# FluxML/Flux3D.jl

Hardware: AMD Instinct MI355X
Metric: chamfer_point_pairs_per_sec (higher is better)
Workload: dtype f32

## Files before the change

flux3d.jl_amd/csrc/chamfer.hip:

```cpp
#include <cmath>
#include <type_traits>

#include "nn1_common.h"

using namespace fx3d;

#ifdef FX3D_PROBE
__device__ unsigned long long g_probe[4096 * 16];
#define FX3D_PROBE_MARK(k)                                                                   \
    do {                                                                                     \
        if (threadIdx.x == 0 && blockIdx.x < 4096) {                                         \
            g_probe[blockIdx.x * 16 + (k)] = __builtin_readcyclecounter();                   \
            if ((k) == 0) g_probe[blockIdx.x * 16 + 13] = wall_clock64();                    \
            if ((k) == 12) g_probe[blockIdx.x * 16 + 14] = wall_clock64();                   \
        }                                                                                    \
    } while (0)
__device__ unsigned long long g_probe2[256 * 16];
#define FX3D_PROBE_MARK2(k) do { if (threadIdx.x == 0 && blockIdx.x < 256) g_probe2[blockIdx.x * 16 + (k)] = __builtin_readcyclecounter(); } while (0)
__device__ unsigned long long g_probe3[16 * 16 * 8];
#define FX3D_PROBE_MARKW(k) do { if ((threadIdx.x & 63) == 0 && blockIdx.x < 16) g_probe3[(blockIdx.x * 16 + (threadIdx.x >> 6)) * 8 + (k)] = __builtin_readcyclecounter(); } while (0)
#else
#define FX3D_PROBE_MARK(k) do { } while (0)
#define FX3D_PROBE_MARK2(k) do { } while (0)
#define FX3D_PROBE_MARKW(k) do { } while (0)
#endif

namespace {

__device__ __forceinline__ void load4pts(const float *__restrict__ base, int p0, float (&px)[4],
                                         float (&py)[4], float (&pz)[4]) {
    const float4 *s4 = reinterpret_cast<const float4 *>(base + (size_t)p0 * 3);
    const float4 f0 = s4[0], f1 = s4[1], f2 = s4[2];
    px[0] = f0.x; py[0] = f0.y; pz[0] = f0.z;
    px[1] = f0.w; py[1] = f1.x; pz[1] = f1.y;
    px[2] = f1.z; py[2] = f1.w; pz[2] = f2.x;
    px[3] = f2.y; py[3] = f2.z; pz[3] = f2.w;
}

typedef _Float16 h8 __attribute__((ext_vector_type(8)));
typedef float f32x16 __attribute__((ext_vector_type(16)));
#ifndef FX3D_HFIFO
#define FX3D_HFIFO 5
#endif
constexpr int kHFifo = FX3D_HFIFO;
#ifndef FX3D_HRUNS_FROM
#define FX3D_HRUNS_FROM 16
#endif
constexpr int kHRunsFrom = FX3D_HRUNS_FROM;
constexpr int kScanU = 2;
#ifndef FX3D_HRUNCAP
#define FX3D_HRUNCAP 384
#endif
constexpr int kHRunCap = FX3D_HRUNCAP;
constexpr int kHItemCap = 64 * kHFifo > kHRunCap ? 64 * kHFifo : kHRunCap;
constexpr int kHFarCap = 64;
#ifndef FX3D_HBLKTRACK
#define FX3D_HBLKTRACK 1
#endif
constexpr bool kHBlkTrack = FX3D_HBLKTRACK != 0;
constexpr int kHIdBits = kHBlkTrack ? 7 : 6;
static_assert(kHChunkMax / (32 * kHLT) <= 64, "lane-tile ids live in the six (block ids: seven) low mantissa bits of the tracked keys");
constexpr float kKeyUp = kHBlkTrack ? 0x1.2p-16f : 0x1.2p-17f;
constexpr float kPadF16 = 65504.0f;
__device__ const unsigned short kHilbertCell[512] = {
    0, 1, 65, 64, 72, 73, 9, 8, 16, 24, 88, 80, 81, 89, 25, 17, 18, 26, 27, 19, 83, 91, 90, 82, 74, 10, 11, 75, 67, 3, 2, 66,
    130, 194, 195, 131, 139, 203, 202, 138, 146, 154, 155, 147, 211, 219, 218, 210, 209, 217, 153, 145, 144, 152, 216, 208, 200, 201, 137, 136, 128, 129, 193, 192,
    256, 257, 265, 264, 328, 329, 321, 320, 384, 448, 456, 392, 393, 457, 449, 385, 386, 450, 451, 387, 395, 459, 458, 394, 330, 322, 323, 331, 267, 259, 258, 266,
    274, 282, 283, 275, 339, 347, 346, 338, 402, 466, 467, 403, 411, 475, 474, 410, 409, 473, 465, 401, 400, 464, 472, 408, 344, 345, 337, 336, 272, 273, 281, 280,
    288, 296, 297, 289, 353, 361, 360, 352, 416, 480, 481, 417, 425, 489, 488, 424, 432, 496, 504, 440, 441, 505, 497, 433, 369, 368, 376, 377, 313, 312, 304, 305,
    306, 307, 315, 314, 378, 379, 371, 370, 434, 498, 506, 442, 443, 507, 499, 435, 427, 491, 490, 426, 418, 482, 483, 419, 355, 363, 362, 354, 290, 298, 299, 291,
    227, 235, 171, 163, 162, 170, 234, 226, 225, 224, 160, 161, 169, 168, 232, 233, 241, 240, 248, 249, 185, 184, 176, 177, 178, 242, 250, 186, 187, 251, 243, 179,
    115, 51, 59, 123, 122, 58, 50, 114, 113, 112, 120, 121, 57, 56, 48, 49, 41, 40, 104, 105, 97, 96, 32, 33, 34, 42, 106, 98, 99, 107, 43, 35,
    36, 44, 108, 100, 101, 109, 45, 37, 38, 39, 103, 102, 110, 111, 47, 46, 54, 55, 63, 62, 126, 127, 119, 118, 117, 53, 61, 125, 124, 60, 52, 116,
    180, 244, 252, 188, 189, 253, 245, 181, 182, 183, 191, 190, 254, 255, 247, 246, 238, 239, 175, 174, 166, 167, 231, 230, 229, 237, 173, 165, 164, 172, 236, 228,
    292, 300, 301, 293, 357, 365, 364, 356, 420, 484, 485, 421, 429, 493, 492, 428, 436, 500, 508, 444, 445, 509, 501, 437, 373, 372, 380, 381, 317, 316, 308, 309,
    310, 311, 319, 318, 382, 383, 375, 374, 438, 502, 510, 446, 447, 511, 503, 439, 431, 495, 494, 430, 422, 486, 487, 423, 359, 367, 366, 358, 294, 302, 303, 295,
    287, 286, 278, 279, 343, 342, 350, 351, 415, 479, 471, 407, 406, 470, 478, 414, 413, 477, 476, 412, 404, 468, 469, 405, 341, 349, 348, 340, 276, 284, 285, 277,
    269, 261, 260, 268, 332, 324, 325, 333, 397, 461, 460, 396, 388, 452, 453, 389, 390, 454, 462, 398, 399, 463, 455, 391, 327, 326, 334, 335, 271, 270, 262, 263,
    199, 198, 134, 135, 143, 142, 206, 207, 215, 223, 159, 151, 150, 158, 222, 214, 213, 221, 220, 212, 148, 156, 157, 149, 141, 205, 204, 140, 132, 196, 197, 133,
    69, 5, 4, 68, 76, 12, 13, 77, 85, 93, 92, 84, 20, 28, 29, 21, 22, 30, 94, 86, 87, 95, 31, 23, 15, 14, 78, 79, 71, 70, 6, 7,
};
constexpr size_t kHScratchBytes = (kHThreads / 64) * (32 * 8 + kHItemCap * 2 + 32 * 3 * 4) + 64 * 32;

__device__ __forceinline__ float vmin(float a, float b) {
    float r;
    asm("v_min_f32 %0, %1, %2" : "=v"(r) : "v"(a), "v"(b));
    return r;
}

__device__ __forceinline__ float vmax(float a, float b) {
    float r;
    asm("v_max_f32 %0, %1, %2" : "=v"(r) : "v"(a), "v"(b));
    return r;
}

__device__ __forceinline__ void split2h(float v, _Float16 &h, _Float16 &l) {
    h = (_Float16)v;
    l = (_Float16)(v - (float)h);
}

constexpr float kBetaC = 0x1.1p-18f;
constexpr float kBandB1 = 1.0f + 18.0f * kBetaC + 0x1p-20f;
constexpr float kBandA = 22.3f * kBetaC + 0x1p-19f;
__device__ __forceinline__ void make_pieces(float cx, float cy, float cz, h8 &p0, h8 &p1) {
    _Float16 hx, lx, hy, ly, hz, lz, n1, n2, n3;
    split2h(cx, hx, lx); split2h(cy, hy, ly); split2h(cz, hz, lz);
    const float n0 = ((cx * cx) + (cy * cy)) + (cz * cz);
    const float n = n0 + kBetaC * n0;
    n1 = (_Float16)n;
    const float r1 = n - (float)n1;
    n2 = (_Float16)r1;
    n3 = (_Float16)(r1 - (float)n2);
    const _Float16 z = (_Float16)0.0f;
    p0 = h8{hx, hx, lx, hy, hy, ly, hz, hz};
    p1 = h8{lz, n1, n2, n3, lx, ly, lz, z};
}

template <bool WANT_IDX, bool SPLITFUSE = false, bool PRUNE = false>
__global__ __launch_bounds__(kHThreads, 4) void nn1_f16_kernel(Nn1Params p) {
    extern __shared__ __attribute__((aligned(16))) float lds[];
    __shared__ __attribute__((aligned(16))) float red[4 * 4 * (kHThreads / 64) + 16];
    __shared__ int nfar[2];
    __shared__ unsigned short farlist[kHFarCap];
    constexpr int QB = (kHThreads / 64) * 32;

    const int L = blockIdx.x;
    const int nsplit = PRUNE ? 1 : p.nsplit;
    const int per_cloud = p.tiles * nsplit;
    const bool by_xcd = 2 * p.B >= 8;
    const int slot = by_xcd ? L >> 3 : L;
    const int c = by_xcd ? (slot / per_cloud) * 8 + (L & 7) : slot / per_cloud;
    const int tile = (slot % per_cloud) / nsplit;
    const int split = (slot % per_cloud) % nsplit;
    if (c >= 2 * p.B) return;
    const int dir = c >= p.B ? 1 : 0;
    const int b = dir ? c - p.B : c;
    const int NQ = dir ? p.M : p.N;
    const int NC = dir ? p.N : p.M;
    if (tile >= (dir ? p.tiles_y : p.tiles_x)) return;
    if ((long long)split * p.chunk >= NC) return;
    const int ctail = (!PRUNE && p.tail > 0 && nsplit == 1 && NC > p.chunk && NC - p.chunk <= p.tail) ? NC - p.chunk : 0;
    const int NCm = NC - ctail;
    const float *__restrict__ qb = (dir ? p.y : p.x) + (size_t)b * NQ * 3;
    const float *__restrict__ cb = (dir ? p.x : p.y) + (size_t)b * NC * 3;
    int32_t *idx_out = dir ? p.idx_y : p.idx_x;
    float *dmin_out = dir ? p.dmin_y : p.dmin_x;

    const int tid = threadIdx.x, lane = tid & 63;
    const int wv = __builtin_amdgcn_readfirstlane(tid >> 6);
    const int jq = lane & 31, hh = lane >> 5;
    const int CH = p.chunk;
    const int tpb = dir ? p.tpb_y : p.tpb;
    h8 *imgp = reinterpret_cast<h8 *>(lds);
    float4 *imgf = reinterpret_cast<float4 *>(lds);
    unsigned long long *wres = reinterpret_cast<unsigned long long *>(lds + 8 * (CH + 64));
    unsigned short *witems = reinterpret_cast<unsigned short *>(wres + (kHThreads / 64) * 32);
    float *wq = reinterpret_cast<float *>(witems + (kHThreads / 64) * kHItemCap);
    unsigned long long *qres = wres + wv * 32;
    unsigned short *items = witems + wv * kHItemCap;
    float *qtab = wq + wv * 96;
    const bool vec = (reinterpret_cast<uintptr_t>(cb) & 15) == 0;
    const bool one_shot = PRUNE || NCm <= CH;
    if (tid == 0) { nfar[0] = 0; nfar[1] = 0; }
    float qpre[3];
    {
        const int q0i = (tile * tpb) * QB + wv * 32 + jq;
        const int qc0 = q0i < NQ ? q0i : NQ - 1;
#pragma unroll
        for (int d = 0; d < 3; ++d) qpre[d] = qb[(size_t)qc0 * 3 + d];
    }
    if constexpr (PRUNE) {
        unsigned int *zc = reinterpret_cast<unsigned int *>(wres);
        for (int i = tid; i < 1040 + 16 * 256; i += kHThreads) zc[i] = 0u;
        int *gb = reinterpret_cast<int *>(wq + (kHThreads / 64) * 96) + 64 * 8;
        for (int i = tid; i < kHGroupsMax * 8; i += kHThreads) gb[i] = (i & 4) ? (int)0x80000000 : 0x7fffffff;
    }
    FX3D_PROBE_MARK(0);

    const bool own_chunk_only = nsplit > 1 && (long long)split * CH + (long long)nsplit * CH >= NCm;
    const int s_lo = own_chunk_only ? split * CH : 0;
    const int SN = own_chunk_only ? (NCm - s_lo < CH ? NCm - s_lo : CH) : NC;
    const float *__restrict__ sb = cb + (size_t)s_lo * 3;
    const bool parked = one_shot || own_chunk_only;
    float mu[3], cinf = 0.0f, varmax = 0.0f;
    float bxlo[3] = {0.f, 0.f, 0.f}, bxhi[3] = {0.f, 0.f, 0.f};
    bool allfin = true;
    {
        float mn[3] = {INFINITY, INFINITY, INFINITY}, mx[3] = {-INFINITY, -INFINITY, -INFINITY}, sm3[3] = {0.f, 0.f, 0.f};
        float sqt = 0.0f;
        const float pil[3] = {sb[0], sb[1], sb[2]};
        const int nsweep = (SN + kHThreads - 1) / kHThreads;
        for (int i0 = 0; i0 < nsweep; i0 += 4) {
            P3 v[4];
#pragma unroll
            for (int e = 0; e < 4; ++e) {
                const int pt = (i0 + e) * kHThreads + tid;
                v[e] = *reinterpret_cast<const P3 *>(sb + (size_t)(pt < SN ? pt : SN - 1) * 3);
            }
#pragma unroll
            for (int e = 0; e < 4; ++e) {
                const int pt = (i0 + e) * kHThreads + tid;
                mn[0] = fminf(mn[0], v[e].x); mx[0] = fmaxf(mx[0], v[e].x);
                mn[1] = fminf(mn[1], v[e].y); mx[1] = fmaxf(mx[1], v[e].y);
                mn[2] = fminf(mn[2], v[e].z); mx[2] = fmaxf(mx[2], v[e].z);
                if (pt < SN) {
                    sm3[0] = sm3[0] + v[e].x; sm3[1] = sm3[1] + v[e].y; sm3[2] = sm3[2] + v[e].z;
                    if (parked) imgf[((pt >> 5) * 2) * 32 + (pt & 31)] = float4{v[e].x, v[e].y, v[e].z, 0.0f};
                }
                if (((i0 + e) & 3) == (wv & 3) && pt < SN) {
                    sqt = __builtin_fmaf(v[e].x - pil[0], v[e].x - pil[0], sqt); sqt = __builtin_fmaf(v[e].y - pil[1], v[e].y - pil[1], sqt);
                    sqt = __builtin_fmaf(v[e].z - pil[2], v[e].z - pil[2], sqt);
                }
            }
        }
        FX3D_PROBE_MARK(5);
        {
            float4 lo4, hi4, st4;
            lo4.x = wave_min_l63(mn[0]); lo4.y = wave_min_l63(mn[1]); lo4.z = wave_min_l63(mn[2]); lo4.w = 0.0f;
            hi4.x = wave_max_l63(mx[0]); hi4.y = wave_max_l63(mx[1]); hi4.z = wave_max_l63(mx[2]); hi4.w = 0.0f;
            st4.x = wave_sum_l63(sm3[0]); st4.y = wave_sum_l63(sm3[1]); st4.z = wave_sum_l63(sm3[2]); st4.w = wave_sum_l63(sqt);
            if (lane == 63) {
                float4 *r4 = reinterpret_cast<float4 *>(red);
                r4[wv * 4] = lo4; r4[wv * 4 + 1] = hi4; r4[wv * 4 + 2] = st4;
            }
        }
        FX3D_PROBE_MARK(9);
        __syncthreads();
        FX3D_PROBE_MARK(10);
        static_assert(kHThreads / 64 == 16, "the cross-wave reduction below: one wave's row of 16 lanes, one lane per wave");
        if (wv == 0) {
            const float4 *r4 = reinterpret_cast<const float4 *>(red);
            const int w = lane & 15;
            float4 lo4 = r4[w * 4], hi4 = r4[w * 4 + 1], st4 = r4[w * 4 + 2];
#define NN1_ROW_MIN(v) v = fkey_inv(row_mm_key<false>(fkey(v)));
#define NN1_ROW_MAX(v) v = fkey_inv(row_mm_key<true>(fkey(v)));
#define NN1_ROW_SUM(v) v = v + dpp_mov<0xB1>(v); v = v + dpp_mov<0x4E>(v); v = v + dpp_mov<0x141>(v); v = v + dpp_mov<0x140>(v);
            NN1_ROW_MIN(lo4.x) NN1_ROW_MIN(lo4.y) NN1_ROW_MIN(lo4.z)
            NN1_ROW_MAX(hi4.x) NN1_ROW_MAX(hi4.y) NN1_ROW_MAX(hi4.z)
            NN1_ROW_SUM(st4.x) NN1_ROW_SUM(st4.y) NN1_ROW_SUM(st4.z) NN1_ROW_SUM(st4.w)
#undef NN1_ROW_MIN
#undef NN1_ROW_MAX
#undef NN1_ROW_SUM
            const float lo3[3] = {lo4.x, lo4.y, lo4.z}, hi3[3] = {hi4.x, hi4.y, hi4.z}, st3[3] = {st4.x, st4.y, st4.z};
            float m3[3], ci = 0.0f, vm = st4.w / fmaxf(0.25f * (float)SN, 1.0f);
            bool fin = true;
#pragma unroll
            for (int d = 0; d < 3; ++d) {
                const float lo = lo3[d], hi = hi3[d], st = st3[d];
                m3[d] = fminf(fmaxf(st / (float)SN, lo), hi);
                const float off = st / (float)SN - pil[d];
                vm = vm - off * off;
                ci = fmaxf(ci, fmaxf(hi - m3[d], m3[d] - lo));
                fin = fin && fabsf(st) < INFINITY;
            }
            if (lane == 0) {
                float4 *o4 = reinterpret_cast<float4 *>(red) + 4 * (kHThreads / 64);
                o4[0] = float4{m3[0], m3[1], m3[2], ci * 1.000001f};
                o4[1] = float4{vm, fin ? 1.0f : 0.0f, 0.0f, 0.0f};
                if (PRUNE) { o4[2] = float4{lo3[0], lo3[1], lo3[2], 0.0f}; o4[3] = float4{hi3[0], hi3[1], hi3[2], 0.0f}; }
            }
        }
        __syncthreads();
        {
            const float4 *o4 = reinterpret_cast<const float4 *>(red) + 4 * (kHThreads / 64);
            const float4 a = o4[0], b2 = o4[1];
            mu[0] = a.x; mu[1] = a.y; mu[2] = a.z; cinf = a.w;
            varmax = b2.x; allfin = b2.y != 0.0f;
            if (PRUNE) {
                const float4 l4 = o4[2], h4 = o4[3];
                bxlo[0] = l4.x; bxlo[1] = l4.y; bxlo[2] = l4.z; bxhi[0] = h4.x; bxhi[1] = h4.y; bxhi[2] = h4.z;
            }
        }
    }
    float rng = cinf;
    if (allfin && cinf < 1.0e16f && 3.0f * cinf * cinf > kRobustGate * varmax) {
        const float4 r = robust_range3<kHThreads, false>(sb, SN, parked, imgf, red, mu[0], mu[1], mu[2], cinf);
        mu[0] = r.x; mu[1] = r.y; mu[2] = r.z; rng = r.w;
    }
    const bool sane = allfin && cinf < 1.0e16f;
    float sc = 1.0f;
    if (sane && rng > 1.0e-30f) {
        int e;
        (void)frexpf(rng, &e);
        sc = ldexpf(1.0f, 7 - e);
    }
    auto uni = [](float v) { return __builtin_bit_cast(float, __builtin_amdgcn_readfirstlane(__builtin_bit_cast(int, v))); };
    mu[0] = uni(mu[0]); mu[1] = uni(mu[1]); mu[2] = uni(mu[2]); sc = uni(sc); rng = uni(rng); cinf = uni(cinf);
    const bool has_far = sane && rng < cinf;
    int fslot = 0;
    auto pieces = [&](float x, float y, float z, int pt, h8 &p0, h8 &p1) {
        const float sx = (x - mu[0]) * sc, sy = (y - mu[1]) * sc, sz = (z - mu[2]) * sc;
        if (!has_far) { make_pieces(sx, sy, sz, p0, p1); return; }
        const bool far = !(fmaxf(fmaxf(fabsf(sx), fabsf(sy)), fabsf(sz)) < 128.0f);
        make_pieces(far ? 0.f : sx, far ? 0.f : sy, far ? 0.f : sz, p0, p1);
        if (far) {
            p1[7] = (_Float16)kPadF16;
            const int f = atomicAdd(&nfar[fslot], 1);
            if (f < kHFarCap) farlist[f] = (unsigned short)pt;
        }
    };

    [[maybe_unused]] float4 *cs = nullptr, *qsw = nullptr;
    [[maybe_unused]] bool sorted_c = false;
    [[maybe_unused]] int qwlen = 0;
    [[maybe_unused]] float4 *boxes = nullptr;
    if constexpr (PRUNE) {
        cs = p.pscr + (size_t)blockIdx.x * p.pscr_stride;
        qsw = cs + kHChunkMax;
        boxes = reinterpret_cast<float4 *>(wq + (kHThreads / 64) * 96);
        unsigned int *ccnt = reinterpret_cast<unsigned int *>(wres);
        unsigned int *qtot = ccnt + 520;
        unsigned int *qwh = qtot + 520;
        const bool last_t = tile == (dir ? p.tiles_y : p.tiles_x) - 1;
        const int qw0 = tile * tpb * QB;
        const int qw1 = last_t || qw0 + tpb * QB > NQ ? NQ : qw0 + tpb * QB;
        qwlen = qw1 - qw0;
        const int cnt = NCm;
        const bool do_sort = sane && cnt >= 512;
        const bool sorted_q = do_sort && NQ <= 4 * kHThreads;
        P3 qv[4];
        if (sorted_q) {
#pragma unroll
            for (int e = 0; e < 4; ++e) {
                const int qp = 256 * wv + 64 * e + lane;
                qv[e] = *reinterpret_cast<const P3 *>(qb + (size_t)(qp < NQ ? qp : NQ - 1) * 3);
            }
        }
        FX3D_PROBE_MARK2(0);
        int *gbox = reinterpret_cast<int *>(boxes + 64 * 2);
        auto group_box = [&](int wrow, float x, float y, float z) {
            int *g = gbox + (wrow >> 5) * 8;
            atomicMin(g + 0, fkey((x - mu[0]) * sc)); atomicMin(g + 1, fkey((y - mu[1]) * sc)); atomicMin(g + 2, fkey((z - mu[2]) * sc));
            atomicMax(g + 4, fkey((x - mu[0]) * sc)); atomicMax(g + 5, fkey((y - mu[1]) * sc)); atomicMax(g + 6, fkey((z - mu[2]) * sc));
        };
        if (do_sort) {
            float4 cv[4];
#pragma unroll
            for (int e = 0; e < 4; ++e) {
                const int pt = e * kHThreads + tid;
                cv[e] = float4{0.f, 0.f, 0.f, 0.f};
                if (pt < cnt) cv[e] = imgf[((pt >> 5) * 2) * 32 + (pt & 31)];
            }
            FX3D_PROBE_MARK2(1);
            float inv[3], off[3], cfl[3], cfh[3];
#pragma unroll
            for (int d = 0; d < 3; ++d) {
                const float fr = has_far ? 0.125f * rng : 128.0f / sc;
                const float flo = fmaxf(bxlo[d], mu[d] - fr), fhi = fminf(bxhi[d], mu[d] + fr);
                inv[d] = fhi > flo ? 8.0f / (fhi - flo) : 0.0f;
                off[d] = -flo * inv[d];
                cfl[d] = flo; cfh[d] = fhi;
            }
            auto cell = [&](float x, float y, float z) -> unsigned int {
                const unsigned int ux = (unsigned int)(int)fminf(fmaxf(__builtin_fmaf(x, inv[0], off[0]), 0.0f), 7.0f);
                const unsigned int uy = (unsigned int)(int)fminf(fmaxf(__builtin_fmaf(y, inv[1], off[1]), 0.0f), 7.0f);
                const unsigned int uz = (unsigned int)(int)fminf(fmaxf(__builtin_fmaf(z, inv[2], off[2]), 0.0f), 7.0f);
                return ux | (uy << 3) | (uz << 6);
            };

            unsigned int ccr[4], qcr[4];
            auto count_cells = [&](bool valid, unsigned int t, auto &&add) -> unsigned int {
                unsigned int rank = 0u;
                bool mine = valid;
                const unsigned int tn = (unsigned int)__builtin_amdgcn_update_dpp((int)~t, (int)t, 0x111, 0xF, 0xF, false);
                if (__builtin_popcountll(__ballot(valid && t == tn)) >= 8) {
                    unsigned long long rem = __ballot(valid);
                    for (int it = 0; it < 12 && rem; ++it) {
                        const unsigned int t0 = (unsigned int)__builtin_amdgcn_readlane((int)t, __builtin_ctzll(rem));
                        const unsigned long long grp = __ballot(mine && t == t0);
                        rem &= ~grp;
                        if (__builtin_popcountll(grp) < 4) continue;
                        unsigned int base = 0u;
                        if ((int)lane == __builtin_ctzll(grp)) base = add(t0, (unsigned int)__builtin_popcountll(grp));
                        base = (unsigned int)__builtin_amdgcn_readlane((int)base, __builtin_ctzll(grp));
                        if (mine && t == t0) {
                            rank = base + __builtin_amdgcn_mbcnt_hi((unsigned int)(grp >> 32), __builtin_amdgcn_mbcnt_lo((unsigned int)grp, 0u));
                            mine = false;
                        }
                    }
                }
                if (mine) rank = add(t, 1u);
                return rank;
            };
#pragma unroll
            for (int e = 0; e < 4; ++e) {
                const int pt = e * kHThreads + tid;
                const unsigned int t = pt < cnt ? cell(cv[e].x, cv[e].y, cv[e].z) : 0u;
                ccr[e] = (t << 16) | count_cells(pt < cnt, t, [&](unsigned int c, unsigned int n) { return atomicAdd(&ccnt[c], n); });
            }
            int *qbb = reinterpret_cast<int *>(boxes + 64 * 2 + kHGroupsMax * 2 - 2);
            if (sorted_q) {
                int kl[3] = {0x7fffffff, 0x7fffffff, 0x7fffffff}, kh[3] = {(int)0x80000000, (int)0x80000000, (int)0x80000000};
#pragma unroll
                for (int e = 0; e < 4; ++e) {
                    const int qp = 256 * wv + 64 * e + lane;
                    if (qp < NQ) {
                        const int k3[3] = {fkey(qv[e].x), fkey(qv[e].y), fkey(qv[e].z)};
#pragma unroll
                        for (int d = 0; d < 3; ++d) { kl[d] = kl[d] < k3[d] ? kl[d] : k3[d]; kh[d] = kh[d] > k3[d] ? kh[d] : k3[d]; }
                    }
                }
#pragma unroll
                for (int d = 0; d < 3; ++d) {
                    int a = row_mm_key<false>(kl[d]), b2 = row_mm_key<true>(kh[d]);
                    a = imm<false>(a, dpp_keepi<0x142, 0xA>(a)); a = imm<false>(a, dpp_keepi<0x143, 0xC>(a));
                    b2 = imm<true>(b2, dpp_keepi<0x142, 0xA>(b2)); b2 = imm<true>(b2, dpp_keepi<0x143, 0xC>(b2));
                    if (lane == 63) { atomicMin(qbb + d, a); atomicMax(qbb + 4 + d, b2); }
                }
            }
            FX3D_PROBE_MARK2(2);
            __syncthreads();
            FX3D_PROBE_MARK2(3);
            float qinv[3] = {0.f, 0.f, 0.f}, qoff[3] = {0.f, 0.f, 0.f};
            if (sorted_q) {
                const float ext = fmaxf(fmaxf(cfh[0] - cfl[0], cfh[1] - cfl[1]), cfh[2] - cfl[2]);
#pragma unroll
                for (int d = 0; d < 3; ++d) {
                    const float ql = fkey_inv(qbb[d]), qh = fkey_inv(qbb[4 + d]);
                    const float grow = qh - ql > 4.0f * ext ? 0.25f * ext : ext;
                    const float lo = fmaxf(ql, cfl[d] - grow), hi = fminf(qh, cfh[d] + grow);
                    qinv[d] = hi > lo && hi - lo < INFINITY ? 8.0f / (hi - lo) : 0.0f;
                    qoff[d] = qinv[d] != 0.0f ? -lo * qinv[d] : 0.0f;
                }
            }
            auto qcell = [&](float x, float y, float z) -> unsigned int {
                const unsigned int ux = (unsigned int)(int)fminf(fmaxf(__builtin_fmaf(x, qinv[0], qoff[0]), 0.0f), 7.0f);
                const unsigned int uy = (unsigned int)(int)fminf(fmaxf(__builtin_fmaf(y, qinv[1], qoff[1]), 0.0f), 7.0f);
                const unsigned int uz = (unsigned int)(int)fminf(fmaxf(__builtin_fmaf(z, qinv[2], qoff[2]), 0.0f), 7.0f);
                return ux | (uy << 3) | (uz << 6);
            };
            auto curve_scan = [&](unsigned int *a) {
                unsigned int tc[8];
                {
                    const uint4 h = *reinterpret_cast<const uint4 *>(kHilbertCell + 8 * lane);
                    tc[0] = h.x & 0xffffu; tc[1] = h.x >> 16; tc[2] = h.y & 0xffffu; tc[3] = h.y >> 16;
                    tc[4] = h.z & 0xffffu; tc[5] = h.z >> 16; tc[6] = h.w & 0xffffu; tc[7] = h.w >> 16;
                }
                unsigned int c8[8], tot = 0u;
#pragma unroll
                for (int k = 0; k < 8; ++k) { c8[k] = a[tc[k]]; tot += c8[k]; }
                unsigned int inc = tot;
#pragma unroll
                for (int o = 1; o < 64; o <<= 1) {
                    const unsigned int v = __shfl_up(inc, o, 64);
                    if (lane >= o) inc += v;
                }
                unsigned int run = inc - tot;
#pragma unroll
                for (int k = 0; k < 8; ++k) { a[tc[k]] = run; run += c8[k]; }
            };
            if (wv == 0) curve_scan(ccnt);
            if (sorted_q) {
#pragma unroll
                for (int e = 0; e < 4; ++e) {
                    const int qp = 256 * wv + 64 * e + lane;
                    const unsigned int t = qp < NQ ? qcell(qv[e].x, qv[e].y, qv[e].z) : 0u;
                    qcr[e] = (t << 16) | count_cells(qp < NQ, t, [&](unsigned int c, unsigned int n) {
                                 const unsigned int sh = 16u * (c & 1u);
                                 const unsigned int old = atomicAdd(&qwh[wv * 256 + (c >> 1)], n << sh);
                                 atomicAdd(&qtot[c], n);
                                 return (old >> sh) & 0xffffu;
                             });
                }
            }
            FX3D_PROBE_MARK2(4);
            __syncthreads();
            FX3D_PROBE_MARK2(5);
#pragma unroll
            for (int e = 0; e < 4; ++e) {
                const int pt = e * kHThreads + tid;
                if (pt < cnt) {
                    const int pos = (int)(ccnt[ccr[e] >> 16] + (ccr[e] & 0xffffu));
                    imgf[((pos >> 5) * 2) * 32 + (pos & 31)] = float4{cv[e].x, cv[e].y, cv[e].z, __builtin_bit_cast(float, pt)};
                }
            }
            sorted_c = true;
            if (sorted_q) {
                if (wv == 1) {
                    curve_scan(qtot);
                } else if (wv >= 2 && wv < 6) {
// ... 22 lines not shown
                            group_box(rank - qw0, qv[e].x, qv[e].y, qv[e].z);
                        }
                    }
                }
            }
        }
        if (!sorted_q) {
            for (int q0 = qw0 + wv * 64; q0 < qw1; q0 += kHThreads) {
                const int qp = q0 + lane;
                const P3 r = *reinterpret_cast<const P3 *>(qb + (size_t)(qp < qw1 ? qp : qw1 - 1) * 3);
                if (qp < qw1) qsw[qp - qw0] = float4{r.x, r.y, r.z, __builtin_bit_cast(float, qp)};
                const int kx = fkey((r.x - mu[0]) * sc), ky = fkey((r.y - mu[1]) * sc), kz = fkey((r.z - mu[2]) * sc);
                const int lx = row_mm_key<false>(kx), ly = row_mm_key<false>(ky), lz = row_mm_key<false>(kz);
                const int hx = row_mm_key<true>(kx), hy = row_mm_key<true>(ky), hz = row_mm_key<true>(kz);
                if ((lane & 15) == 0 && qp < qw1) {
                    int *g = gbox + ((qp - qw0) >> 5) * 8;
                    atomicMin(g + 0, lx); atomicMin(g + 1, ly); atomicMin(g + 2, lz);
                    atomicMax(g + 4, hx); atomicMax(g + 5, hy); atomicMax(g + 6, hz);
                }
            }
        }
        FX3D_PROBE_MARK2(8);
    }
    FX3D_PROBE_MARK(1);

    const float cm2 = 3.0f * (fminf(cinf * sc, 128.0f) * fminf(cinf * sc, 128.0f));
    float qr[3], da = 0.0f;
    float da_far = 0.0f;
    [[maybe_unused]] float dpr = INFINITY;
    bool qfin = true;
    int qi = 0;
    bool qok = true;
    h8 bq;
    double acc = 0.0;

    const int jfirst = split * CH, jstep = nsplit * CH;
    for (int j0 = jfirst; j0 < NCm; j0 += jstep) {
        const int cnt = PRUNE || (NCm - j0) < CH ? (NCm - j0) : CH;
        const bool last_chunk = PRUNE || j0 + jstep >= NCm;
        const int cnt_pad = (cnt + 32 * kHLT - 1) / (32 * kHLT) * (32 * kHLT);
        if (j0 > jfirst) __syncthreads();
        if constexpr (PRUNE) {
            auto stage_tile = [&](int tl, auto full_c) {
                constexpr bool kFull = decltype(full_c)::value;
                float4 r4[4];
#pragma unroll
                for (int k = 0; k < 4; ++k) {
                    const int pt = tl * 64 + k * 16 + (tid & 15);
                    if (!kFull) r4[k] = float4{0.f, 0.f, 0.f, 0.f};
                    if (kFull || pt < cnt) r4[k] = imgf[((pt >> 5) * 2) * 32 + (pt & 31)];
                }
                float lo3[3] = {INFINITY, INFINITY, INFINITY}, hi3[3] = {-INFINITY, -INFINITY, -INFINITY};
#pragma unroll
                for (int k = 0; k < 4; ++k) {
                    const int pt = tl * 64 + k * 16 + (tid & 15), i0 = ((pt >> 5) * 2) * 32 + (pt & 31);
                    h8 p0, p1;
                    if (kFull || pt < cnt) {
                        pieces(r4[k].x, r4[k].y, r4[k].z, pt, p0, p1);
                        const int id = sorted_c ? __builtin_bit_cast(int, r4[k].w) : j0 + pt;
                        cs[pt] = float4{r4[k].x, r4[k].y, r4[k].z, __builtin_bit_cast(float, id)};
                        const float b3[3] = {(r4[k].x - mu[0]) * sc, (r4[k].y - mu[1]) * sc, (r4[k].z - mu[2]) * sc};
#pragma unroll
                        for (int d = 0; d < 3; ++d) { lo3[d] = vmin(lo3[d], b3[d]); hi3[d] = vmax(hi3[d], b3[d]); }
                    } else {
                        make_pieces(0.f, 0.f, 0.f, p0, p1);
                        p1[7] = (_Float16)kPadF16;
                    }
                    imgp[i0] = p0;
                    imgp[i0 + 32] = p1;
                }
                float bl[3], bh[3];
#pragma unroll
                for (int d = 0; d < 3; ++d) { bl[d] = fkey_inv(row_mm_key<false>(fkey(lo3[d]))); bh[d] = fkey_inv(row_mm_key<true>(fkey(hi3[d]))); }
                if ((tid & 15) == 0 && tl < 64) {
                    boxes[tl * 2] = float4{bl[0], bl[1], bl[2], 0.0f};
                    boxes[tl * 2 + 1] = float4{bh[0], bh[1], bh[2], 0.0f};
                }
            };
            for (int tw = 4 * wv; tw * 64 < cnt_pad + 64; tw += kHThreads / 16) {
                const int tl = tw + (lane >> 4);
                if (64 * (tw + 4) <= cnt) {
                    stage_tile(tl, std::true_type{});
                } else if (64 * tw < cnt) {
                    if (tl * 64 < cnt_pad + 64) stage_tile(tl, std::false_type{});
                } else if (tl * 64 < cnt_pad + 64) {
                    h8 p0, p1;
                    make_pieces(0.f, 0.f, 0.f, p0, p1);
                    p1[7] = (_Float16)kPadF16;
#pragma unroll
                    for (int k = 0; k < 4; ++k) {
                        const int pt = tl * 64 + k * 16 + (tid & 15), i0 = ((pt >> 5) * 2) * 32 + (pt & 31);
                        imgp[i0] = p0;
                        imgp[i0 + 32] = p1;
                    }
                    if ((tid & 15) == 0 && tl < 64) {
                        boxes[tl * 2] = float4{INFINITY, INFINITY, INFINITY, 0.0f};
                        boxes[tl * 2 + 1] = float4{-INFINITY, -INFINITY, -INFINITY, 0.0f};
                    }
                }
            }
        } else
        for (int pt = tid; pt < cnt_pad + 64; pt += kHThreads) {
            const int i0 = ((pt >> 5) * 2) * 32 + (pt & 31);
            h8 p0, p1;
            if (pt < cnt) {
                if (parked) {
                    const float4 r = imgf[i0];
                    pieces(r.x, r.y, r.z, pt, p0, p1);
                } else {
                    const P3 r = *reinterpret_cast<const P3 *>(cb + (size_t)(j0 + pt) * 3);
                    pieces(r.x, r.y, r.z, pt, p0, p1);
                }
            } else {
                make_pieces(0.f, 0.f, 0.f, p0, p1);
                p1[7] = (_Float16)kPadF16;
            }
            imgp[i0] = p0;
            imgp[i0 + 32] = p1;
        }
        __syncthreads();
        FX3D_PROBE_MARK(j0 == jfirst ? 2 : 6);
        FX3D_PROBE_MARKW(0);

        const int nf = nfar[fslot];
        if constexpr (!PRUNE) {
            if (tid == 0) nfar[fslot ^ 1] = 0;
            fslot ^= 1;
        }
        const bool far_ok = nf <= kHFarCap;
        const bool last_tile = tile == (dir ? p.tiles_y : p.tiles_x) - 1;
        for (int tp = 0; tp < tpb || (last_tile && one_shot); ++tp) {
            if ((tile * tpb + tp) * QB >= NQ) break;
            if constexpr (PRUNE) {
                if (tp * QB + wv * 32 >= qwlen) continue;
            }
            if (j0 == jfirst) {
                qi = (tile * tpb + tp) * QB + wv * 32 + jq;
                if constexpr (PRUNE) {
                    const int wpos = tp * QB + wv * 32 + jq;
                    const float4 q4 = qsw[wpos < qwlen ? wpos : qwlen - 1];
                    qr[0] = q4.x; qr[1] = q4.y; qr[2] = q4.z;
                    qi = wpos < qwlen ? __builtin_bit_cast(int, q4.w) : NQ;
                } else if (tp == 0) {
#pragma unroll
                    for (int d = 0; d < 3; ++d) qr[d] = qpre[d];
                } else {
                    const int qc1 = qi < NQ ? qi : NQ - 1;
#pragma unroll
                    for (int d = 0; d < 3; ++d) qr[d] = qb[(size_t)qc1 * 3 + d];
                }
                float m0 = -2.0f * ((qr[0] - mu[0]) * sc), m1 = -2.0f * ((qr[1] - mu[1]) * sc), m2 = -2.0f * ((qr[2] - mu[2]) * sc);
                float S = (fabsf(m0) + fabsf(m1)) + fabsf(m2);
                float sq = 1.0f, fl_s = 0.0f;
                if (S >= 3.0e4f && S < 0x1p28f) {
                    int e;
                    (void)frexpf(S, &e);
                    sq = ldexpf(1.0f, 14 - e);
                    m0 *= sq; m1 *= sq; m2 *= sq; S *= sq;
                    fl_s = 0x1p-15f;
                }
                qok = S < 3.0e4f;
                qfin = fabsf(qr[0]) + fabsf(qr[1]) + fabsf(qr[2]) < INFINITY;
                const float qn = 0.25f * ((m0 * m0 + m1 * m1) + m2 * m2) / sq;
                da = kBandA * qn + 0x1p-24f * (S + 4.0f) + fl_s;
                {
                    const float c2 = sq * cm2;
                    da_far = 2.1f * kBetaC * c2 + 2.0f * kBetaC * sqrtf(qn * c2) + 0x1p-19f * qn + 0x1p-24f * (S + 4.0f) + fl_s;
                }
                if constexpr (PRUNE) {
                    dpr = qok && sq == 1.0f ? qn + 2.0f * kBetaC * (cm2 + qn) + 0x1p-23f * (S + 4.0f) : INFINITY;
                }
                _Float16 hx, lx, hy, ly, hz, lz;
                split2h(qok ? m0 : 0.f, hx, lx); split2h(qok ? m1 : 0.f, hy, ly); split2h(qok ? m2 : 0.f, hz, lz);
                const _Float16 one = (_Float16)sq, pad = (_Float16)kPadF16;
                bq = hh == 0 ? h8{hx, lx, hx, hy, ly, hy, hz, lz} : h8{hz, one, one, one, lx, ly, lz, pad};
                if (hh == 0) {
                    qres[jq] = ~0ull;
                    qtab[jq * 3 + 0] = qr[0]; qtab[jq * 3 + 1] = qr[1]; qtab[jq * 3 + 2] = qr[2];
                }
            }

            float tm = INFINITY, fk[kHFifo];
#pragma unroll
            for (int s = 0; s < kHFifo; ++s) fk[s] = INFINITY;
            const unsigned int keymask = ~((1u << kHIdBits) - 1u);

            static_assert(kHLT == 2, "the rotation below is written for lane tiles of two blocks");
            const int nblk = cnt_pad / 32;
            f32x16 zero;
#pragma unroll
            for (int r = 0; r < 16; ++r) zero[r] = 0.0f;
#define NN1_FOLD(ACC, FIRST)                                                                                         \
            {                                                                                                        \
                const float t0 = min3f(ACC[0], ACC[1], ACC[2]), t1 = min3f(ACC[3], ACC[4], ACC[5]);                  \
                const float t2 = min3f(ACC[6], ACC[7], ACC[8]), t3 = min3f(ACC[9], ACC[10], ACC[11]);                \
                const float t4 = min3f(ACC[12], ACC[13], ACC[14]);                                                   \
                const float t5 = min3f(t0, t1, t2), t6 = min3f(t3, t4, ACC[15]);                                     \
                tm = (FIRST) ? vmin(t5, t6) : min3f(tm, t5, t6);       \
            }
#define NN1_TRACK_ID(LT)                                                                                             \
            {                                                                                                        \
                float key;                                                                                           \
                asm("v_and_or_b32 %0, %1, %2, %3" : "=v"(key) : "v"(tm), "v"(keymask), "s"(LT));                     \
                _Pragma("unroll") for (int s_ = kHFifo - 1; s_ > 0; --s_) fk[s_] = __builtin_amdgcn_fmed3f(fk[s_ - 1], fk[s_], key);    \
                fk[0] = vmin(fk[0], key);                                                                            \
            }
#define NN1_TRACK() { NN1_TRACK_ID(lt) ++lt; }
#define NN1_CLOSE(ACC, ODD, LT)                                                                                      \
            if constexpr (kHBlkTrack) { NN1_FOLD(ACC, true) NN1_TRACK_ID(2 * (LT) + (ODD)) }                           \
            else { NN1_FOLD(ACC, !(ODD)) if (ODD) NN1_TRACK_ID(LT) }
#define NN1_STEP(ISSUE, FOLD, ODD, OFF)                                                                              \
            __builtin_amdgcn_s_setprio(0);                                                                           \
            ISSUE = __builtin_amdgcn_mfma_f32_32x32x16_f16(an, bq, zero, 0, 0, 0);                                   \
            an = pa[(OFF) * 64];                                                                                     \
            __builtin_amdgcn_s_setprio(1);                                                                           \
            NN1_CLOSE(FOLD, ODD, lt)                                                                                 \
            if (ODD) ++lt;
            if constexpr (!PRUNE) {
            const h8 *pa = imgp + hh * 32 + jq;
            f32x16 acc0, acc1, acc2;
            h8 an = pa[0];
            acc0 = __builtin_amdgcn_mfma_f32_32x32x16_f16(an, bq, zero, 0, 0, 0); an = pa[1 * 64];
            acc1 = __builtin_amdgcn_mfma_f32_32x32x16_f16(an, bq, zero, 0, 0, 0); an = pa[2 * 64];
            pa += 3 * 64;
            int lt = 0;
            int nb = 2;
            for (; nb + 6 <= nblk; nb += 6) {
                NN1_STEP(acc2, acc0, 0, 0) NN1_STEP(acc0, acc1, 1, 1) NN1_STEP(acc1, acc2, 0, 2)
                NN1_STEP(acc2, acc0, 1, 3) NN1_STEP(acc0, acc1, 0, 4) NN1_STEP(acc1, acc2, 1, 5)
                pa += 6 * 64;
            }
            if (nblk - nb == 4) {
                NN1_STEP(acc2, acc0, 0, 0) NN1_STEP(acc0, acc1, 1, 1) NN1_STEP(acc1, acc2, 0, 2) NN1_STEP(acc2, acc0, 1, 3)
                NN1_CLOSE(acc1, 0, lt) NN1_CLOSE(acc2, 1, lt)
            } else if (nblk - nb == 2) {
                NN1_STEP(acc2, acc0, 0, 0) NN1_STEP(acc0, acc1, 1, 1)
                NN1_CLOSE(acc2, 0, lt) NN1_CLOSE(acc0, 1, lt)
            } else {
                NN1_CLOSE(acc0, 0, lt) NN1_CLOSE(acc1, 1, lt)
            }
            } else {
            const int nltp = nblk / kHLT;
            float bd = INFINITY;
            {
                const int4 *gq = reinterpret_cast<const int4 *>(boxes + 64 * 2) + (tp * (kHThreads / 64) + wv) * 2;
                const int4 gl = gq[0], gh = gq[1];
                const float qlx = fkey_inv(gl.x), qly = fkey_inv(gl.y), qlz = fkey_inv(gl.z);
                const float qhx = fkey_inv(gh.x), qhy = fkey_inv(gh.y), qhz = fkey_inv(gh.z);
                if (lane < nltp) {
                    const float4 lo = boxes[lane * 2], hi = boxes[lane * 2 + 1];
                    const float gx = fmaxf(fmaxf(lo.x - qhx, qlx - hi.x), 0.0f), gy = fmaxf(fmaxf(lo.y - qhy, qly - hi.y), 0.0f);
                    const float gz = fmaxf(fmaxf(lo.z - qhz, qlz - hi.z), 0.0f);
                    bd = (gx * gx + gy * gy) + gz * gz;
                }
            }
            const unsigned long long all_lt = nltp >= 64 ? ~0ull : (1ull << nltp) - 1ull;
            unsigned long long todo = all_lt, done = 0ull;
            if (sorted_c) {
                todo = __ballot(bd == 0.0f);
                if (!todo) {
                    const float bmin = wave_min_f(bd);
                    todo = bmin < INFINITY ? __ballot(bd == bmin) : all_lt;
                }
            }
            const h8 *pbase = imgp + hh * 32 + jq;
            for (int phase = 0; phase < 2; ++phase) {
                if (phase == 1) {
                    if (done == all_lt) break;
                    const float kb = fk[0];
                    const float bb = __builtin_fmaf(fabsf(kb), kKeyUp, kb);
                    const float dj = fminf(bb, __shfl_xor(bb, 32, 64)) + dpr;
                    const float ucut = wave_max_f(__builtin_fmaf(dj, 1.0f + 0x1p-9f, 0x1p-8f));
                    const bool keep = !(bd > ucut) || !(dj == dj);
                    todo = (__ballot(!(dj == dj)) ? all_lt : __ballot(keep)) & all_lt & ~done;
                    if (!todo) break;
                }
                done |= todo;
                unsigned long long mk = todo;
                int nrem = __builtin_popcountll(mk) - 1;
#define NN1_NEXT(T) { T = nltp; if (mk) { T = __builtin_ctzll(mk); mk &= mk - 1ull; } }
                int ta, tb;
                NN1_NEXT(ta) NN1_NEXT(tb)
                f32x16 acc0, acc1, acc2;
                const h8 *pn = pbase + ta * (kHLT * 64);
                h8 an = pn[0];
                acc0 = __builtin_amdgcn_mfma_f32_32x32x16_f16(an, bq, zero, 0, 0, 0); an = pn[64];
                pn = pbase + tb * (kHLT * 64);
                acc1 = __builtin_amdgcn_mfma_f32_32x32x16_f16(an, bq, zero, 0, 0, 0); an = pn[0];
#define NN1_PSTEP(ISSUE, FOLD, ODD, LT, NEXT)                                                                         \
                __builtin_amdgcn_s_setprio(0);                                                                       \
                ISSUE = __builtin_amdgcn_mfma_f32_32x32x16_f16(an, bq, zero, 0, 0, 0);                               \
                an = NEXT;                                                                                           \
                __builtin_amdgcn_s_setprio(1);                                                                       \
                NN1_CLOSE(FOLD, ODD, LT)
                while (nrem >= 3) {
                    int tc, td, te;
                    NN1_NEXT(tc) NN1_NEXT(td) NN1_NEXT(te)
                    nrem -= 3;
                    const h8 *pc = pbase + tc * (kHLT * 64), *pd = pbase + td * (kHLT * 64);
                    NN1_PSTEP(acc2, acc0, 0, ta, pn[64])
                    NN1_PSTEP(acc0, acc1, 1, ta, pc[0])
                    pn = pbase + te * (kHLT * 64);
                    NN1_PSTEP(acc1, acc2, 0, tb, pc[64])
                    NN1_PSTEP(acc2, acc0, 1, tb, pd[0])
                    NN1_PSTEP(acc0, acc1, 0, tc, pd[64])
                    NN1_PSTEP(acc1, acc2, 1, tc, pn[0])
                    ta = td; tb = te;
                }
                if (nrem == 2) {
                    int tc;
                    NN1_NEXT(tc)
                    const h8 *pc = pbase + tc * (kHLT * 64);
                    NN1_PSTEP(acc2, acc0, 0, ta, pn[64])
                    NN1_PSTEP(acc0, acc1, 1, ta, pc[0])
                    NN1_PSTEP(acc1, acc2, 0, tb, pc[64])
                    NN1_PSTEP(acc2, acc0, 1, tb, pc[64])
                    NN1_CLOSE(acc1, 0, tc) NN1_CLOSE(acc2, 1, tc)
                } else if (nrem == 1) {
                    NN1_PSTEP(acc2, acc0, 0, ta, pn[64])
                    NN1_PSTEP(acc0, acc1, 1, ta, pn[64])
                    NN1_CLOSE(acc2, 0, tb) NN1_CLOSE(acc0, 1, tb)
                } else {
                    NN1_CLOSE(acc0, 0, ta) NN1_CLOSE(acc1, 1, ta)
                }
#undef NN1_PSTEP
#undef NN1_NEXT
                __builtin_amdgcn_s_setprio(0);
#ifdef FX3D_PROBE_COUNT
                if ((threadIdx.x & 63) == 0) atomicAdd(&g_probe[4095 * 16 + 6 + phase], (unsigned long long)__builtin_popcountll(todo));
#endif
            }
            }
#undef NN1_STEP
#undef NN1_CLOSE
#undef NN1_TRACK
#undef NN1_TRACK_ID
#undef NN1_FOLD
            __builtin_amdgcn_s_setprio(0);
            float ft[kHFifo];
#pragma unroll
            for (int s = 0; s < kHFifo; ++s) ft[s] = fk[s];
            const float ka = fk[0];
            const float best = __builtin_fmaf(fabsf(ka), kKeyUp, ka);
            FX3D_PROBE_MARK(tp == 0 ? 3 : 7);
            FX3D_PROBE_MARKW(tp == 0 ? 1 : 3);

            {
                int opq;
                asm volatile("s_mov_b32 %0, 0" : "=s"(opq));
                const int lane = (int)(threadIdx.x & 63) + opq, jq = lane & 31, hh = lane >> 5;
                const float m = fminf(best, __shfl_xor(best, 32, 64));
                const float thr1 = fminf(__builtin_fmaf(m, kBandB1, da), __builtin_fmaf(m, 1.0f + 0x1p-20f, da_far));
                const float thr1k = __builtin_fmaf(fabsf(thr1), kKeyUp, thr1);
                const bool usable = sane && far_ok && qok && m < INFINITY;
                const bool slow = !usable || !(fk[kHFifo - 1] > thr1k);
                const unsigned long long sb = __ballot(slow);
                unsigned int qslow = (unsigned int)sb | (unsigned int)(sb >> 32);
                const bool retry = __builtin_popcount(qslow) > 2;
                bool fifo_done = false;
                const bool nonfinite = !sane || __ballot(!qfin) != 0;
                const int nlt = nblk / kHLT;
                int lt2 = 0;
                const bool runs = retry && __builtin_popcount(qslow) >= kHRunsFrom;
#ifdef FX3D_PROBE_COUNT
                if ((threadIdx.x & 63) == 0) {
                    unsigned long long *pc = &g_probe[4095 * 16];
                    atomicAdd(&pc[0], 1ull); atomicAdd(&pc[1], qslow ? 1ull : 0ull); atomicAdd(&pc[2], retry ? 1ull : 0ull);
                    atomicAdd(&pc[3], runs ? 1ull : 0ull); atomicAdd(&pc[4], (unsigned long long)__builtin_popcount(qslow));
                    atomicAdd(&pc[5], (unsigned long long)__builtin_popcountll(__ballot(!usable)));
                }
#endif
                const int lt2_end = runs ? nblk : nlt;
                do {
                    int nitems = 0;
                    if (!retry && fifo_done) {
                        const int qsl = __builtin_ctz(qslow);
                        qslow &= qslow - 1;
                        const float qq[3] = {qtab[qsl * 3], qtab[qsl * 3 + 1], qtab[qsl * 3 + 2]};
                        unsigned long long kbest = ~0ull;
                        for (int h = 0; h < 2; ++h) {
                            if (!((sb >> (32 * h + qsl)) & 1ull)) continue;
                            for (int r0 = 4 * (2 * lane + h); r0 < cnt; r0 += kScanU * 512) {
                                float cx[kScanU][4], cy[kScanU][4], cz[kScanU][4];
                                [[maybe_unused]] int cid[kScanU][4];
#pragma unroll
                                for (int u = 0; u < kScanU; ++u) {
                                    const int jl0 = r0 + 512 * u;
                                    if constexpr (PRUNE) {
#pragma unroll
                                        for (int r = 0; r < 4; ++r) {
                                            const float4 v = cs[jl0 + r < cnt ? jl0 + r : cnt - 1];
                                            cx[u][r] = v.x; cy[u][r] = v.y; cz[u][r] = v.z; cid[u][r] = __builtin_bit_cast(int, v.w);
                                        }
                                    } else if (vec && jl0 + 4 <= cnt) {
                                        load4pts(cb, j0 + jl0, cx[u], cy[u], cz[u]);
                                    } else {
#pragma unroll
                                        for (int r = 0; r < 4; ++r) {
                                            const int jc = jl0 + r < cnt ? jl0 + r : cnt - 1;
                                            const float *src = cb + (size_t)(j0 + jc) * 3;
                                            cx[u][r] = src[0]; cy[u][r] = src[1]; cz[u][r] = src[2];
                                        }
                                    }
                                }
#pragma unroll
                                for (int u = 0; u < kScanU; ++u)
#pragma unroll
                                    for (int r = 0; r < 4; ++r) {
                                        const int jc = r0 + 512 * u + r;
                                        const float cc3[3] = {cx[u][r], cy[u][r], cz[u][r]};
                                        const unsigned int cidx = PRUNE ? (unsigned int)cid[u][r] : (unsigned int)(j0 + jc);
                                        const unsigned long long key = ((unsigned long long)dist_key(sqd<3>(qq, cc3)) << 32) | cidx;
                                        if (jc < cnt && key < kbest) kbest = key;
                                    }
                            }
                        }
                        atomicMin(&qres[qsl], kbest);
                        lt2 = qslow ? 0 : nlt;
                    } else if (!retry) {
#pragma unroll
                        for (int s = 0; s < kHFifo; ++s) {
                            const bool qual = ft[s] <= thr1k;
                            const unsigned long long bal = __ballot(qual);
                            if (bal) {
                                const int pos = nitems + __builtin_amdgcn_mbcnt_hi((unsigned int)(bal >> 32),
                                                         __builtin_amdgcn_mbcnt_lo((unsigned int)bal, 0));
                                if (qual) items[pos] = (unsigned short)(((unsigned int)jq << (kHIdBits + 1)) | ((unsigned int)hh << kHIdBits) |
                                                                        (__builtin_bit_cast(unsigned int, ft[s]) & ((1u << kHIdBits) - 1u)));
                                nitems += __builtin_popcountll(bal);
                            }
                        }
                        fifo_done = true;
                        lt2 = qslow ? 0 : nlt;
                    } else {
                        const h8 *pb = imgp + hh * 32 + jq;
                        if (!runs) {
#pragma unroll 1
                            for (; lt2 < nlt && nitems <= kHItemCap - 64 * kHLT; ++lt2) {
                                float t2 = INFINITY;
#pragma unroll
                                for (int bb = 0; bb < kHLT; ++bb) {
                                    const f32x16 av = __builtin_amdgcn_mfma_f32_32x32x16_f16(pb[(lt2 * kHLT + bb) * 64], bq, zero, 0, 0, 0);
                                    if (kHBlkTrack) t2 = INFINITY;
#pragma unroll
                                    for (int r = 0; r < 16; r += 2) t2 = min3f(t2, av[r], av[r + 1]);
                                    if (kHBlkTrack || bb == kHLT - 1) {
                                        const bool qual = !usable || t2 <= thr1;
                                        const unsigned long long bal = __ballot(qual);
                                        if (bal) {
                                            const int pos = nitems + __builtin_amdgcn_mbcnt_hi((unsigned int)(bal >> 32),
                                                                     __builtin_amdgcn_mbcnt_lo((unsigned int)bal, 0));
                                            const unsigned int id = kHBlkTrack ? (unsigned int)(lt2 * kHLT + bb) : (unsigned int)lt2;
                                            if (qual) items[pos] = (unsigned short)(((unsigned int)jq << (kHIdBits + 1)) | ((unsigned int)hh << kHIdBits) | id);
                                            nitems += __builtin_popcountll(bal);
                                        }
                                    }
                                }
                            }
                        } else
#pragma unroll 1
                        for (; lt2 < nblk && nitems <= kHItemCap - 256; ++lt2) {
                            const f32x16 av = __builtin_amdgcn_mfma_f32_32x32x16_f16(pb[lt2 * 64], bq, zero, 0, 0, 0);
#pragma unroll
                            for (int g = 0; g < 4; ++g) {
                                const float mg = vmin(min3f(av[4 * g], av[4 * g + 1], av[4 * g + 2]), av[4 * g + 3]);
                                const bool qual = !usable || mg <= thr1;
                                const unsigned long long bal = __ballot(qual);
                                if (bal) {
                                    const int pos = nitems + __builtin_amdgcn_mbcnt_hi((unsigned int)(bal >> 32),
                                                             __builtin_amdgcn_mbcnt_lo((unsigned int)bal, 0));
                                    if (qual) items[pos] = (unsigned short)(((unsigned int)jq << 10) | ((unsigned int)hh << 9) | ((unsigned int)lt2 << 2) | (unsigned int)g);
                                    nitems += __builtin_popcountll(bal);
                                }
                            }
                        }
                    }
                    __builtin_amdgcn_s_waitcnt(0xc07f);
                    __builtin_amdgcn_wave_barrier();
                    if (!runs) {
                    constexpr int kRunsPerItem = kHBlkTrack ? 4 : kHLT * 4;
                    const int ntask = nitems * kRunsPerItem;
                    for (int t0 = 0; t0 < ntask; t0 += 64) {
                        const int t = t0 + lane;
                        if (t < ntask) {
                            const unsigned int it = items[t / kRunsPerItem];
                            const int run = t % kRunsPerItem;
                            const int qs = it >> (kHIdBits + 1), ih = (it >> kHIdBits) & 1, tl = it & ((1u << kHIdBits) - 1u);
                            const int jl0 = kHBlkTrack ? tl * 32 + 8 * run + 4 * ih : (tl * kHLT + (run >> 2)) * 32 + 8 * (run & 3) + 4 * ih;
                            float cx[4], cy[4], cz[4];
                            [[maybe_unused]] int cid[4];
                            if constexpr (PRUNE) {
#pragma unroll
                                for (int r = 0; r < 4; ++r) {
                                    const float4 v = cs[jl0 + r];
                                    cx[r] = v.x; cy[r] = v.y; cz[r] = v.z; cid[r] = __builtin_bit_cast(int, v.w);
                                }
                            } else if (vec && jl0 + 4 <= cnt) {
                                load4pts(cb, j0 + jl0, cx, cy, cz);
                            } else {
#pragma unroll
                                for (int r = 0; r < 4; ++r) {
                                    const int jc = jl0 + r < cnt ? jl0 + r : cnt - 1;
                                    const float *src = cb + (size_t)(j0 + jc) * 3;
                                    cx[r] = src[0]; cy[r] = src[1]; cz[r] = src[2];
                                }
                            }
                            const float qq[3] = {qtab[qs * 3], qtab[qs * 3 + 1], qtab[qs * 3 + 2]};
                            unsigned int kb;
                            int ib = j0 + jl0;
                            if constexpr (PRUNE) {
                                unsigned long long k64 = ~0ull;
                                if (!nonfinite) {
#pragma unroll
                                    for (int r = 0; r < 4; ++r) {
                                        const float cc3[3] = {cx[r], cy[r], cz[r]};
                                        const unsigned long long key = ((unsigned long long)__builtin_bit_cast(unsigned int, sqd<3>(qq, cc3)) << 32) | (unsigned int)cid[r];
                                        if (jl0 + r < cnt && key < k64) k64 = key;
                                    }
                                } else {
#pragma unroll
                                    for (int r = 0; r < 4; ++r) {
                                        const float cc3[3] = {cx[r], cy[r], cz[r]};
                                        const unsigned long long key = ((unsigned long long)dist_key(sqd<3>(qq, cc3)) << 32) | (unsigned int)cid[r];
                                        if (jl0 + r < cnt && key < k64) k64 = key;
                                    }
                                }
                                kb = (unsigned int)(k64 >> 32); ib = (int)(unsigned int)k64;
                            } else
                            if (!nonfinite) {
                                float db = INFINITY;
#pragma unroll
                                for (int r = 0; r < 4; ++r) {
                                    const float cc3[3] = {cx[r], cy[r], cz[r]};
                                    const float dd = sqd<3>(qq, cc3);
                                    if (jl0 + r < cnt && dd < db) { db = dd; ib = j0 + jl0 + r; }
                                }
                                kb = __builtin_bit_cast(unsigned int, db);
                            } else {
                                kb = 0xffffffffu;
#pragma unroll
                                for (int r = 0; r < 4; ++r) {
                                    const float cc3[3] = {cx[r], cy[r], cz[r]};
                                    const unsigned int kd = dist_key(sqd<3>(qq, cc3));
                                    if (jl0 + r < cnt && kd < kb) { kb = kd; ib = j0 + jl0 + r; }
                                }
                            }
                            if (jl0 < cnt) atomicMin(&qres[qs], ((unsigned long long)kb << 32) | (unsigned int)ib);
                        }
                    }
                    } else {
#pragma unroll 1
                        for (int t0 = 0; t0 < nitems; t0 += 64) {
                            const int t = t0 + lane;
                            if (t < nitems) {
                                const unsigned int it = items[t];
                                const int qs = (int)(it >> 10);
                                const int jl0 = (int)((it >> 2) & 127u) * 32 + 8 * (int)(it & 3u) + 4 * (int)((it >> 9) & 1u);
                                const float qq[3] = {qtab[qs * 3], qtab[qs * 3 + 1], qtab[qs * 3 + 2]};
                                unsigned long long kbest = ~0ull;
#pragma unroll
                                for (int r = 0; r < 4; ++r) {
                                    const int jc = jl0 + r < cnt ? jl0 + r : cnt - 1;
                                    float cc3[3];
                                    unsigned int cidx = (unsigned int)(j0 + jc);
                                    if constexpr (PRUNE) {
                                        const float4 v = cs[jc];
                                        cc3[0] = v.x; cc3[1] = v.y; cc3[2] = v.z; cidx = __builtin_bit_cast(unsigned int, v.w);
                                    } else {
                                        const float *src = cb + (size_t)(j0 + jc) * 3;
                                        cc3[0] = src[0]; cc3[1] = src[1]; cc3[2] = src[2];
                                    }
                                    const unsigned long long key = ((unsigned long long)dist_key(sqd<3>(qq, cc3)) << 32) | cidx;
                                    if (jl0 + r < cnt && key < kbest) kbest = key;
                                }
                                if (jl0 < cnt) atomicMin(&qres[qs], kbest);
                            }
                        }
                    }
                } while (lt2 < lt2_end);
                if (far_ok) {
                    for (int t = lane; t < 32 * nf; t += 64) {
                        const int qs = t & 31, jc = farlist[t >> 5];
                        const float qq[3] = {qtab[qs * 3], qtab[qs * 3 + 1], qtab[qs * 3 + 2]};
                        float cc3[3];
                        unsigned int cidx = (unsigned int)(j0 + jc);
                        if constexpr (PRUNE) {
                            const float4 v = cs[jc];
                            cc3[0] = v.x; cc3[1] = v.y; cc3[2] = v.z; cidx = __builtin_bit_cast(unsigned int, v.w);
                        } else {
                            const float *src = cb + (size_t)(j0 + jc) * 3;
                            cc3[0] = src[0]; cc3[1] = src[1]; cc3[2] = src[2];
                        }
                        const float dd = sqd<3>(qq, cc3);
                        const unsigned int kd = nonfinite ? dist_key(dd) : __builtin_bit_cast(unsigned int, dd);
                        atomicMin(&qres[qs], ((unsigned long long)kd << 32) | cidx);
                    }
                }
                if (ctail && last_chunk) {
                    for (int t = lane; t < 32 * ctail; t += 64) {
                        const int qs = t & 31, jc = NCm + (t >> 5);
                        const float qq[3] = {qtab[qs * 3], qtab[qs * 3 + 1], qtab[qs * 3 + 2]};
                        const float *src = cb + (size_t)jc * 3;
                        const float cc3[3] = {src[0], src[1], src[2]};
                        atomicMin(&qres[qs], ((unsigned long long)dist_key(sqd<3>(qq, cc3)) << 32) | (unsigned int)jc);
                    }
                }
            }
            FX3D_PROBE_MARK(tp == 0 ? 4 : 8);
            FX3D_PROBE_MARKW(tp == 0 ? 2 : 4);

            if (last_chunk) {
                __builtin_amdgcn_s_waitcnt(0xc07f);
                __builtin_amdgcn_wave_barrier();
                if (hh == 0) {
                    const unsigned long long r = qres[jq];
                    const float dd = __builtin_bit_cast(float, (unsigned int)(r >> 32));
                    const int ii = (int)(unsigned int)r;
                    if (nsplit > 1) {
                        unsigned long long *gp = &p.gres[((size_t)split * 2 * p.B + c) * p.qstride + qi];
                        if (qi < NQ) {
                            if (SPLITFUSE) __hip_atomic_store(gp, r, __ATOMIC_RELAXED, __HIP_MEMORY_SCOPE_AGENT);
                            else *gp = r;
                        }
                    } else if (qi < NQ) {
                        if (WANT_IDX && idx_out) idx_out[(size_t)b * NQ + qi] = ii;
                        if (dmin_out) dmin_out[(size_t)b * NQ + qi] = dd;
                        acc += (double)dd;
                    }
                }
// ... 155 lines not shown
```

Before: 15280 billion.

## Hoist query preload, replace divisions and wave max with cheaper variants

Moves the sorted-query preload earlier in the PRUNE path so its global loads are issued before the reductions and can overlap with them. Replaces a division by the power-of-two scale with multiplication by a precomputed reciprocal. Uses the raw hardware sqrt with a small upward fudge in the PRUNE path. Replaces the wave-wide float max with a row-reduction on integer keys plus readlanes. It also adds a probe counter and changes an epsilon threshold, which brings extra register pressure and slight numeric changes.

```diff
diff --git a/flux3d.jl_amd/csrc/chamfer.hip b/flux3d.jl_amd/csrc/chamfer.hip
--- a/flux3d.jl_amd/csrc/chamfer.hip
+++ b/flux3d.jl_amd/csrc/chamfer.hip
@@ -162,12 +162,22 @@
     const bool vec = (reinterpret_cast<uintptr_t>(cb) & 15) == 0;
     const bool one_shot = PRUNE || NCm <= CH;
     if (tid == 0) { nfar[0] = 0; nfar[1] = 0; }
-    float qpre[3];
-    {
+    [[maybe_unused]] float qpre[3];
+    if constexpr (!PRUNE) {
         const int q0i = (tile * tpb) * QB + wv * 32 + jq;
         const int qc0 = q0i < NQ ? q0i : NQ - 1;
 #pragma unroll
         for (int d = 0; d < 3; ++d) qpre[d] = qb[(size_t)qc0 * 3 + d];
+    }
+    [[maybe_unused]] P3 qv[4];
+    if constexpr (PRUNE) {
+        if (NQ <= 4 * kHThreads) {
+#pragma unroll
+            for (int e = 0; e < 4; ++e) {
+                const int qp = 256 * wv + 64 * e + lane;
+                qv[e] = *reinterpret_cast<const P3 *>(qb + (size_t)(qp < NQ ? qp : NQ - 1) * 3);
+            }
+        }
     }
     if constexpr (PRUNE) {
         unsigned int *zc = reinterpret_cast<unsigned int *>(wres);
@@ -279,7 +289,7 @@
     }
     const bool sane = allfin && cinf < 1.0e16f;
     float sc = 1.0f;
-    if (sane && rng > 1.0e-30f) {
+    if (sane && rng > 0x1p-50f) {
         int e;
         (void)frexpf(rng, &e);
         sc = ldexpf(1.0f, 7 - e);
@@ -318,14 +328,6 @@
         const int cnt = NCm;
         const bool do_sort = sane && cnt >= 512;
         const bool sorted_q = do_sort && NQ <= 4 * kHThreads;
-        P3 qv[4];
-        if (sorted_q) {
-#pragma unroll
-            for (int e = 0; e < 4; ++e) {
-                const int qp = 256 * wv + 64 * e + lane;
-                qv[e] = *reinterpret_cast<const P3 *>(qb + (size_t)(qp < NQ ? qp : NQ - 1) * 3);
-            }
-        }
         FX3D_PROBE_MARK2(0);
         int *gbox = reinterpret_cast<int *>(boxes + 64 * 2);
         auto group_box = [&](int wrow, float x, float y, float z) {
@@ -654,20 +656,25 @@
                 float m0 = -2.0f * ((qr[0] - mu[0]) * sc), m1 = -2.0f * ((qr[1] - mu[1]) * sc), m2 = -2.0f * ((qr[2] - mu[2]) * sc);
                 float S = (fabsf(m0) + fabsf(m1)) + fabsf(m2);
                 float sq = 1.0f, fl_s = 0.0f;
+                float rsq = 1.0f;
                 if (S >= 3.0e4f && S < 0x1p28f) {
                     int e;
                     (void)frexpf(S, &e);
                     sq = ldexpf(1.0f, 14 - e);
+                    rsq = ldexpf(1.0f, e - 14);
                     m0 *= sq; m1 *= sq; m2 *= sq; S *= sq;
                     fl_s = 0x1p-15f;
                 }
                 qok = S < 3.0e4f;
                 qfin = fabsf(qr[0]) + fabsf(qr[1]) + fabsf(qr[2]) < INFINITY;
-                const float qn = 0.25f * ((m0 * m0 + m1 * m1) + m2 * m2) / sq;
+                const float qn = 0.25f * ((m0 * m0 + m1 * m1) + m2 * m2) * rsq;
                 da = kBandA * qn + 0x1p-24f * (S + 4.0f) + fl_s;
                 {
                     const float c2 = sq * cm2;
-                    da_far = 2.1f * kBetaC * c2 + 2.0f * kBetaC * sqrtf(qn * c2) + 0x1p-19f * qn + 0x1p-24f * (S + 4.0f) + fl_s;
+                    float root;
+                    if constexpr (PRUNE) root = __builtin_fmaf(__builtin_amdgcn_sqrtf(qn * c2), 1.0f + 0x1p-20f, 0x1p-62f);
+                    else root = sqrtf(qn * c2);
+                    da_far = 2.1f * kBetaC * c2 + 2.0f * kBetaC * root + 0x1p-19f * qn + 0x1p-24f * (S + 4.0f) + fl_s;
                 }
                 if constexpr (PRUNE) {
                     dpr = qok && sq == 1.0f ? qn + 2.0f * kBetaC * (cm2 + qn) + 0x1p-23f * (S + 4.0f) : INFINITY;
@@ -771,8 +778,10 @@
                     if (done == all_lt) break;
                     const float kb = fk[0];
                     const float bb = __builtin_fmaf(fabsf(kb), kKeyUp, kb);
-                    const float dj = fminf(bb, __shfl_xor(bb, 32, 64)) + dpr;
-                    const float ucut = wave_max_f(__builtin_fmaf(dj, 1.0f + 0x1p-9f, 0x1p-8f));
+                    const float dj = vmin(bb, __shfl_xor(bb, 32, 64)) + dpr;
+                    const int kr = row_mm_key<true>(fkey(__builtin_fmaf(dj, 1.0f + 0x1p-9f, 0x1p-8f)));
+                    const float ucut = fkey_inv(imm<true>(imm<true>(__builtin_amdgcn_readlane(kr, 0), __builtin_amdgcn_readlane(kr, 16)),
+                                                          imm<true>(__builtin_amdgcn_readlane(kr, 32), __builtin_amdgcn_readlane(kr, 48))));
                     const bool keep = !(bd > ucut) || !(dj == dj);
                     todo = (__ballot(!(dj == dj)) ? all_lt : __ballot(keep)) & all_lt & ~done;
                     if (!todo) break;
@@ -977,6 +986,9 @@
                             }
                         }
                     }
+#ifdef FX3D_PROBE_COUNT
+                    if ((threadIdx.x & 63) == 0) atomicAdd(&g_probe[4095 * 16 + 8], (unsigned long long)nitems);
+#endif
                     __builtin_amdgcn_s_waitcnt(0xc07f);
                     __builtin_amdgcn_wave_barrier();
                     if (!runs) {
```

Measured after the change: 15440 billion, median of 6. 1.0% higher.
